# Guilucand/PanDelos

Measured on AMD Instinct MI355X. Metric: scored gene-pairs/sec (whole node), higher is better.
Workload: dtype u32 accumulate + f32 finalize

## Files before the change

### pandelos_amd/csrc/pdl_api.hip

```cpp
#include "pdl_common.h"

#include <algorithm>
#include <cstdlib>
#include <cstring>
#include <limits>

static thread_local std::string g_create_error = "";

#define PDL_GUARD_BEGIN try {
#define PDL_GUARD_END(ctx_)                                                       \
    } catch (const pdl_error &e) {                                                \
        if (ctx_) (ctx_)->err = e.msg; else g_create_error = e.msg;               \
        return e.code;                                                            \
    } catch (const std::bad_alloc &) {                                            \
        if (ctx_) (ctx_)->err = "host allocation failed";                         \
        return PDL_ERR_DEVICE;                                                    \
    }

template <class T> static T *xalloc(size_t n) {
    T *p = static_cast<T *>(malloc((n ? n : 1) * sizeof(T)));
    if (!p) throw std::bad_alloc();
    return p;
}

// ... 543 lines not shown
        if ((n_edges && (!src || !dst)) || (n_sequences && !genome_of)) PDL_FAIL(PDL_ERR_ARGUMENT, "pdl_families_of_edges: NULL pointer");
        if (n_edges >= 0x7fffffffull || n_sequences >= 0x7fffffffu) PDL_FAIL(PDL_ERR_UNSUPPORTED, "pdl_families_of_edges: 2^31 genes or edges and more");
        PDL_HIP(hipSetDevice(c->device));
        pdl_ctx::FamBufs &b = c->fb;
        uint32_t g_max = 0;
        for (uint32_t i = 0; i < n_sequences; i++) g_max = std::max(g_max, genome_of[i]);
        if (n_edges) {
            b.up_src.alloc(n_edges * 4); b.up_dst.alloc(n_edges * 4);
            PDL_HIP(hipMemcpyAsync(b.up_src.p, src, n_edges * 4, hipMemcpyHostToDevice, c->stream));
            PDL_HIP(hipMemcpyAsync(b.up_dst.p, dst, n_edges * 4, hipMemcpyHostToDevice, c->stream));
        }
        if (n_sequences) {
            b.up_gen.alloc((size_t) n_sequences * 4);
            PDL_HIP(hipMemcpyAsync(b.up_gen.p, genome_of, (size_t) n_sequences * 4, hipMemcpyHostToDevice, c->stream));
        }
        const int32_t *s2[2] = {b.up_src.as<int32_t>(), nullptr}, *d2[2] = {b.up_dst.as<int32_t>(), nullptr};
        const uint64_t n2[2] = {n_edges, 0};
        pdl_fam_result r;
        pdl_run_families(c, s2, d2, n2, false, true, true, b.up_gen.as<uint32_t>(), n_sequences, bit_length64(g_max), r);
        fill_families(r, out);
        return PDL_OK;
    } catch (const pdl_error &e) { c->err = e.msg; pdl_free_families(out); return e.code;
    } catch (const std::bad_alloc &) { c->err = "host allocation failed"; pdl_free_families(out); return PDL_ERR_DEVICE; }
}

int pdl_set_option(pdl_ctx *c, const char *name, int64_t value) {
    if (!c || !name) return PDL_ERR_ARGUMENT;
    std::lock_guard<std::mutex> lk(c->mu);
    const std::string n(name);
    if (n == "join_tier1") {
        if (!(value == -1 || value == 0 || (value >= 9 && value <= 11) || value == 20 || value == 21)) { c->err = "join_tier1: -1, 0, 9, 10, 11, 20 or 21"; return PDL_ERR_ARGUMENT; }
        c->opt_tier1 = (int) value;
    } else if (n == "join_tier0") c->opt_tier0 = value < 0 ? -1 : (value != 0);
    else if (n == "join_tiny_tier2") c->opt_tiny_tier2 = value != 0;
    else if (n == "join_grid_pct") c->opt_grid_pct = (int) value;
    else if (n == "stage_timers") c->opt_stage_timers = value != 0;
    else if (n == "host_mirror") c->opt_host_mirror = value != 0;
    else if (n == "staging_cap") c->opt_staging_cap = value > 0 ? (uint64_t) value : 0;
    else if (n == "aside_test_reload") c->opt_aside_test_reload = value != 0;
    else if (n == "onepass_scan") c->opt_onepass_scan = value != 0;
    else if (n == "low_memory") c->opt_low_memory = value != 0;
    else if (n == "query_batch_bytes") {
        if (value <= 0) { c->err = "query_batch_bytes: a positive byte count"; return PDL_ERR_ARGUMENT; }
        c->opt_query_batch_bytes = (uint64_t) value;
        return PDL_OK;
    }
    else { c->err = "unknown option " + n; return PDL_ERR_ARGUMENT; }
    c->scored = false;
    return PDL_OK;
}

int pdl_dist_preprocess_begin(pdl_ctx *c, const uint8_t *d_residues, const uint64_t *d_offsets, const uint32_t *d_genome_of,
                              uint32_t n, uint64_t n_res, int k, uint32_t world, uint32_t rank, pdl_dist_slice *out) {
    if (!c || !out) return PDL_ERR_ARGUMENT;
    std::lock_guard<std::mutex> lk(c->mu);
    PDL_GUARD_BEGIN
    if (!d_offsets || !d_genome_of || (!d_residues && n_res)) PDL_FAIL(PDL_ERR_ARGUMENT, "null input pointer");
    if (((uintptr_t) d_residues & 15) != 0) PDL_FAIL(PDL_ERR_ARGUMENT, "d_residues must be 16-byte aligned");
    if (world == 0 || rank >= world || world > 64) PDL_FAIL(PDL_ERR_ARGUMENT, "rank %u of %u (at most 64 ranks)", rank, world);
    PDL_HIP(hipSetDevice(c->device));
    c->preprocessed = false; c->scored = false; c->tasks_ready = false; c->mirror_valid = false;
    c->dist = false; c->dist_stage = 0;
    adopt_device_input(c, d_residues, d_offsets, d_genome_of, n, n_res);
    c->N = n; c->R = n_res;
    c->U = c->Ushared = c->NG = c->P = c->M = 0;
    if (k <= 0) PDL_FAIL(PDL_ERR_KVALUE, "K value must be greater than 0.");
// ... 281 lines not shown
```

### pandelos_amd/csrc/pdl_common.h

```cpp
#pragma once

#include <atomic>
#include <chrono>

#include <hip/hip_runtime.h>

#include <cstdint>
#include <cstdio>
#include <mutex>
#include <cstdlib>
#include <string>
#include <utility>
#include <vector>

#include "../../include/pandelos_amd.h"

#define PDL_WAVE 64

#ifdef __HIPCC__
__device__ __forceinline__ void pdl_sync() {
#ifndef PDL_PLAIN_SYNCTHREADS
    asm volatile("s_waitcnt lgkmcnt(0)" ::: "memory");
#endif
    __syncthreads();
// ... 227 lines not shown
    bool scored = false;
    uint32_t n_task_rows = 0;
    std::vector<int32_t> h_local_genome;
    std::vector<uint32_t> h_task_row_off;
    std::vector<uint64_t> h_cell_off;
    DevBuf task_blob;
    uint32_t *task_pin = nullptr; size_t task_pin_words = 0;
    hipStream_t copy_stream = nullptr; hipEvent_t ev_tasks = nullptr, ev_entry = nullptr;
    DevView task_rows;
    DevView task_lg;
    DevBuf row_desc;
    DevBuf MS;
    DevBuf CM;
    DevBuf row_base, row_cnt, fin_off;
    DevBuf st_score, st_perc, st_tr, st_col, st_first;
    uint64_t st_cap = 0;
    DevBuf c_score, c_perc, c_tr, c_row, c_col;
    uint64_t Z = 0;
    DevBuf join_ctr;
    DevBuf overflow_rows;
    DevBuf gene_info;
    DevBuf join_defer;
    DevBuf glb_table;
    bool glb_clean = false;
    DevBuf row_desc2;
    DevBuf mirror_cnt, mirror_ref;
    DevView taskpos_of;
    std::vector<uint32_t> h_fin;
    bool tasks_ready = false;
    DevBuf scratch2;
    DevBuf task_off;
    int cus = 0;
    uint32_t occ_tier1[5] = {0, 0, 0, 0, 0};
    uint32_t occ_tier0 = 0, occ_tier0b = 0;

    bool edges_valid = false;
    DevBuf bbh_kind, bbh_tab, e_src, e_dst, e_score;
    uint8_t *edge_mirror = nullptr;
    size_t edge_mirror_bytes = 0;
    uint64_t n_edges = 0, n_edges1 = 0;
    std::vector<uint32_t> h_bbh_at;
    std::vector<uint64_t> h_edge1, h_edge_off;

    int opt_tier1 = -1;
    int opt_tier0 = -1;
    bool opt_tiny_tier2 = false;
    bool opt_stage_timers = true;
    int opt_grid_pct = 0;
    bool opt_host_mirror = true;
    uint64_t opt_staging_cap = 0;
    bool opt_aside_test_reload = false;

    bool dist = false;
    uint32_t world = 1, rank = 0;
    int dist_stage = 0;
    uint2 *post_ext = nullptr;
    uint64_t U_slice = 0, M_slice = 0;
    std::vector<uint32_t> h_owner;
    std::vector<uint64_t> h_upper_cost;
    std::vector<uint64_t> h_run_weights;
    std::vector<uint64_t> h_run_costs;
    bool dist_sender = false;
    int dist_tail = -1;
    uint64_t run_base = 0, dist_total = 0;
    DevBuf seq_owner;
    DevBuf tuple_off;
    std::vector<uint64_t> h_tuple_counts;
    uint32_t *dist_out_keys = nullptr;
    unsigned long long *dist_out_ranges = nullptr;
    uint64_t dist_out_total = 0, dist_run_counters[3] = {0, 0, 0};
    DevBuf owner_of_genome;
    DevView local_genome;
    DevBuf outbox;
    DevBuf outbox_tab;
    std::vector<uint64_t> h_outbox_counts;
    uint64_t st_local = 0;
    uint64_t n_inbox = 0;
    uint32_t order_grid1 = 0;
// ... 226 lines not shown
```

### pandelos_amd/csrc/pdl_join.hip

```cpp
#include "pdl_common.h"
#include "pdl_scan.h"

#include <algorithm>
#include <cstdlib>
#include <cstring>

constexpr int HBM_THREADS = 512;
constexpr uint32_t EMPTY_KEY = 0xffffffffu;
constexpr uint64_t FIELD_MASK = (1ull << 21) - 1;
constexpr uint32_t CELL_CHUNK = 16384;

struct JoinArgs {
    const uint2 *post;
    const uint4 *ranges;
    const uint2 *ranges8;
    const uint32_t *seq_off;
    const uint32_t *kseq_len;
    const uint32_t *genome_of;
    const uint4 *gene_info;
    const uint32_t *task_rows;
    const uint32_t *task_lg;
    const uint32_t *work;
    const uint4 *desc;
    uint32_t n_work;
    const uint32_t *n_work_ptr;
    uint32_t N, G, k;
    uint32_t min_kseq;
    uint32_t canonical;
    float *MS;
    float *CM;
    uint32_t *row_base, *row_cnt;
    float *st_score, *st_perc, *st_tr;
    uint32_t *st_col, *st_first;
    uint32_t mirror;
    const uint32_t *taskpos_of;
    const uint32_t *local_genome;
    uint32_t *mirror_cnt;
    unsigned long long st_cap;
    uint32_t *work_cursor;
    uint32_t work_batch;
    unsigned long long *cell_cursor;
    uint32_t *overflow_count;
    uint32_t *error_count;
    uint32_t *overflow_rows;
    uint4 *overflow_desc;
#ifdef PDL_JOIN_PHASES
    unsigned long long *phase;
#endif
    void *defer;
    uint32_t defer_wide;
    uint32_t defer_cap;
    uint32_t *reload_count;
    uint32_t defer_serial;
    unsigned long long *hbm_acc;
    uint32_t *hbm_u32;
};

__device__ __forceinline__ uint32_t min_numerator(float threshold, float denom) {
    uint32_t n = (uint32_t) (threshold * denom);
    n = n > 2 ? n - 2 : 0;
    while ((float) (int) n / denom < threshold) n++;
    return n;
}

__device__ __forceinline__ float finalize_counts(int inter, int pc, int tc, uint32_t my_kcnt, uint32_t other_kcnt, float threshold,
                                                 float &perc, float &tr_perc) {
    const int union_size = (int) my_kcnt + (int) other_kcnt - inter;
    perc = (float) pc / (float) (int) my_kcnt;
    tr_perc = (float) tc / (float) (int) other_kcnt;
    const bool score_valid = perc >= threshold || tr_perc >= threshold;
    return (float) inter / (float) union_size * (score_valid ? 1.0f : 0.0f);
}
__device__ __forceinline__ float finalize_cell(unsigned long long acc, uint32_t my_kcnt, uint32_t other_kcnt, float threshold,
// ... 1098 lines not shown
        const uint32_t g = c->shard[i];
        c->h_local_genome[g] = (int32_t) i;
        c->h_task_row_off[i] = p;
        for (uint32_t j = c->h_genome_row_off[g]; j < c->h_genome_row_off[g + 1]; j++) { const uint32_t gene = c->h_genome_rows[j]; h_rows[p] = gene; h_lg[p] = i; h_pos[gene] = p; p++; }
    }
    for (uint32_t g = 0; g < G; g++) h_loc[g] = (uint32_t) c->h_local_genome[g];
    c->h_task_row_off[S] = n_rows;
    c->n_task_rows = n_rows;
    c->tasks_ready = true;
    if (!c->copy_stream) {
        PDL_HIP(hipStreamCreateWithFlags(&c->copy_stream, hipStreamNonBlocking));
        PDL_HIP(hipEventCreateWithFlags(&c->ev_tasks, hipEventDisableTiming));
    }
    memcpy(c->task_pin + words, c->h_task_row_off.data(), (size_t) (S + 1) * 4);
    c->task_blob.alloc(words * sizeof(uint32_t) + 16);
    if (n_rows) c->task_off.alloc((size_t) (S + 1) * 8 + 96);
    PDL_HIP(hipMemcpyAsync(c->task_blob.p, c->task_pin, words * sizeof(uint32_t), hipMemcpyHostToDevice, c->copy_stream));
    if (n_rows) PDL_HIP(hipMemcpyAsync(c->task_off.p, c->task_pin + words, (size_t) (S + 1) * 4, hipMemcpyHostToDevice, c->copy_stream));
    PDL_HIP(hipEventRecord(c->ev_tasks, c->copy_stream));
    PDL_HIP(hipStreamWaitEvent(st, c->ev_tasks, 0));
    uint32_t *d = c->task_blob.as<uint32_t>();
    c->task_rows.p = d; c->task_lg.p = d + n_rows; c->taskpos_of.p = d + 2 * (size_t) n_rows; c->local_genome.p = d + 2 * (size_t) n_rows + N;
    if (c->dist) {
        c->owner_of_genome.alloc((size_t) G * 4);
        PDL_HIP(hipMemcpyAsync(c->owner_of_genome.p, c->h_owner.data(), (size_t) G * 4, hipMemcpyHostToDevice, st));
    }
}

__global__ void k_iota_u32(uint32_t *dst, uint32_t n) { uint32_t i = blockIdx.x * blockDim.x + threadIdx.x; if (i < n) dst[i] = i; }

struct ScorePlan {
    bool wide, mirror;
    bool tier0;
    uint32_t grid0, grid0b;
    int tier1, occ_slot;
    bool tiny_tier2;
    uint32_t grid1, grid2, grid3;
    unsigned long long slack;
    bool wide_aside;
};

static ScorePlan score_plan(pdl_ctx *c) {
    const uint32_t N = c->N, G = c->G;
    const uint32_t n_rows = c->n_task_rows;
    const uint32_t S = (uint32_t) c->shard.size();
    ScorePlan pl{};
    pl.wide = c->max_kseq >= (1ull << 20);
    if (c->max_kseq >= (1ull << 31)) PDL_FAIL(PDL_ERR_UNSUPPORTED, "a gene with %llu k-mers exceeds the reference's int counters", (unsigned long long) c->max_kseq);
    pl.mirror = c->upper_only;
    if (pl.mirror && !c->dist && (c->shard_set && S != G))
        PDL_FAIL(PDL_ERR_STATE, "the dictionary was built for all genomes (upper-triangle ranges); a genome shard must be set before pdl_preprocess");
    const int cus = pdl_cus(c);
    pl.tier1 = c->opt_tier1 >= 0 ? c->opt_tier1 : (G <= 320 ? 10 : 11);
    pl.tiny_tier2 = c->opt_tiny_tier2;
    auto occupancy = [&](const void *fn, int threads) {
        int nb = 0;
        if (hipOccupancyMaxActiveBlocksPerMultiprocessor(&nb, fn, threads, 0) != hipSuccess || nb < 1) nb = 1;
        return (uint32_t) nb;
    };
    const int tier1 = pl.tier1;
    const void *fn1 = tier1 == 9 ? (const void *) k_join_lds<9, 128, true>
                    : tier1 == 10 ? (const void *) k_join_lds<10, 256, true>
                    : tier1 == 11 ? (const void *) k_join_lds<11, 256, true>
                    : tier1 == 20 ? (const void *) k_join_lds<10, 256, false> : (const void *) k_join_lds<11, 256, false>;
    const int t1_threads = tier1 == 9 ? 128 : 256;
    pl.occ_slot = tier1 >= 20 ? tier1 - 20 + 3 : (tier1 ? tier1 - 9 : 0);
    if (tier1 && c->occ_tier1[pl.occ_slot] == 0) c->occ_tier1[pl.occ_slot] = occupancy(fn1, t1_threads);
    pl.grid1 = tier1 ? std::min<uint32_t>(n_rows, (uint32_t) cus * c->occ_tier1[pl.occ_slot]) : 0;
    if (c->opt_grid_pct > 0 && pl.grid1) pl.grid1 = std::max<uint32_t>(1, (uint32_t) ((uint64_t) pl.grid1 * (uint32_t) c->opt_grid_pct / 100));
    {
        const unsigned long long walked = c->dist ? [&] { unsigned long long u = 0; for (uint32_t g : c->shard) u += c->h_upper_cost[g]; return u; }()
                                          : pl.mirror ? (c->P - c->Ushared) / 2 : c->P;
        const bool can = c->ranges8 != nullptr && !pl.wide && c->min_kseq > 2ull * c->rp.k && tier1 != 0;
        const bool want = c->opt_tier0 > 0 || (c->opt_tier0 < 0 && c->opt_tier1 < 0 && n_rows >= 12288 && walked / n_rows <= 3000 && c->Urepeat * 5000 <= c->U);
        pl.tier0 = can && want;
        if (pl.tier0) {
            if (c->occ_tier0 == 0) { c->occ_tier0 = occupancy((const void *) k_join_part<PT_T, PT_WG_PER_CU>, (int) PT_T); c->occ_tier0b = occupancy((const void *) k_join_part<PT_T2, PT_WGS2>, (int) PT_T2); }
            pl.grid0 = std::min<uint32_t>((n_rows + PT_BATCH - 1) / PT_BATCH, (uint32_t) cus * c->occ_tier0);
            pl.grid0b = std::min<uint32_t>(n_rows, (uint32_t) cus * c->occ_tier0b);
            if (c->opt_grid_pct > 0) pl.grid0 = std::max<uint32_t>(1, (uint32_t) ((uint64_t) pl.grid0 * (uint32_t) c->opt_grid_pct / 100));
        }
    }
    pl.grid2 = std::min<uint32_t>(n_rows, (uint32_t) cus * (pl.tiny_tier2 ? 4 : 1));
    {
        const unsigned long long per_wg = (unsigned long long) std::max<uint32_t>(N, 1) * ((pl.wide ? 2 : 1) * sizeof(uint64_t) + 3 * sizeof(uint32_t));
        const unsigned long long fit = ((c->opt_low_memory ? 1ull : 8ull) << 30) / per_wg;
        pl.grid3 = (uint32_t) std::min<unsigned long long>((unsigned long long) cus, std::max<unsigned long long>(64, fit));
    }
    const size_t hbm_bytes = (size_t) pl.grid3 * N * ((pl.wide ? 2 : 1) * sizeof(uint64_t) + 3 * sizeof(uint32_t));
    if (c->glb_table.bytes < hbm_bytes) { c->glb_table.alloc(hbm_bytes); c->glb_clean = false; }
    if (!c->glb_clean) {
        PDL_HIP(hipMemsetAsync(c->glb_table.p, 0, hbm_bytes, c->stream));
        c->glb_clean = true;
    }
    pl.slack = 2ull * (pl.grid0 + pl.grid0b + pl.grid1 + pl.grid2 + pl.grid3) * CELL_CHUNK;
    return pl;
}

static void score_alloc_rows(pdl_ctx *c, const ScorePlan &pl) {
    const uint32_t N = c->N, G = c->G, n_rows = c->n_task_rows;
    const uint32_t S = (uint32_t) c->shard.size();
    c->MS.alloc((size_t) n_rows * G * sizeof(float) + 16);
    c->CM.alloc((size_t) S * N * sizeof(float) + 16);
    c->row_base.alloc((size_t) n_rows * 4); c->row_cnt.alloc((size_t) n_rows * 4); c->fin_off.alloc(((size_t) n_rows + 2) * 4);
    c->join_ctr.alloc(PDL_JC_WORDS * sizeof(uint32_t));
    c->row_desc.alloc((size_t) n_rows * sizeof(uint4));
    c->row_desc2.alloc((size_t) n_rows * sizeof(uint4) * (pl.tier0 ? 3 : 1));
    c->overflow_rows.alloc((size_t) n_rows * 4 * 4);
    if (pl.mirror) c->mirror_cnt.alloc((size_t) n_rows * 4 * 3 + 16);
    c->gene_info.alloc((size_t) N * sizeof(uint4));
    hipLaunchKernelGGL(k_row_desc, dim3((std::max(n_rows, N) + 255) / 256), dim3(256), 0, c->stream, c->task_rows.as<uint32_t>(), c->seq_off.as<uint32_t>(),
                       n_rows, c->row_desc.as<uint4>(), c->kseq_len.as<uint32_t>(), c->d_gen, c->taskpos_of.as<uint32_t>(), c->local_genome.as<uint32_t>(),
                       N, c->gene_info.as<uint4>());
}

static void score_alloc_cells(pdl_ctx *c, const ScorePlan &pl, unsigned long long cap, unsigned long long extra) {
    const unsigned long long fcap = pl.mirror ? 2 * cap + extra : cap;
    if (fcap >= 0xffffffffull) PDL_FAIL(PDL_ERR_UNSUPPORTED, "more than 2^32 emitted cells on one device: shard the genomes over more devices");
    DevBuf *st[5] = {&c->st_score, &c->st_perc, &c->st_tr, &c->st_col, &c->st_first};
    for (int i = 0; i < 5; i++) st[i]->alloc(cap * 4);
    c->c_score.alloc(fcap * 4); c->c_perc.alloc(fcap * 4); c->c_tr.alloc(fcap * 4); c->c_row.alloc(fcap * 4); c->c_col.alloc(fcap * 4);
    if (pl.mirror) c->mirror_ref.alloc((cap + extra) * sizeof(MCell));
    c->st_cap = cap;
}

static JoinArgs join_args(pdl_ctx *c, const ScorePlan &pl) {
    JoinArgs a{};
    a.post = pdl_postings(c); a.ranges = c->ranges.as<uint4>(); a.ranges8 = c->ranges8; a.seq_off = c->seq_off.as<uint32_t>();
    a.kseq_len = c->kseq_len.as<uint32_t>(); a.genome_of = c->d_gen; a.gene_info = c->gene_info.as<uint4>();
    a.task_rows = c->task_rows.as<uint32_t>(); a.task_lg = c->task_lg.as<uint32_t>();
    a.N = c->N; a.G = c->G; a.k = c->rp.k;
    a.min_kseq = (uint32_t) std::max<uint64_t>(c->min_kseq, 1); a.canonical = (c->flags & PDL_FLAG_CANONICAL_ORDER) ? 1u : 0u;
    a.MS = c->MS.as<float>(); a.CM = c->CM.as<float>();
    a.row_base = c->row_base.as<uint32_t>(); a.row_cnt = c->row_cnt.as<uint32_t>();
    a.st_score = c->st_score.as<float>(); a.st_perc = c->st_perc.as<float>(); a.st_tr = c->st_tr.as<float>();
    a.st_col = c->st_col.as<uint32_t>(); a.st_first = c->st_first.as<uint32_t>(); a.st_cap = c->st_cap;
    a.mirror = pl.mirror ? 1u : 0u;
    if (pl.mirror) {
        a.taskpos_of = c->taskpos_of.as<uint32_t>(); a.local_genome = c->local_genome.as<uint32_t>();
        a.mirror_cnt = c->mirror_cnt.as<uint32_t>();
    }
    return a;
}

static void score_join(pdl_ctx *c, const ScorePlan &pl) {
    hipStream_t st = c->stream;
    const uint32_t N = c->N, G = c->G, n_rows = c->n_task_rows;
    const uint32_t S = (uint32_t) c->shard.size();
    const int tier1 = pl.tier1;
    {
        auto n16 = [](size_t bytes) { return (unsigned long long) ((bytes + 15) / 16); };
        ZeroRanges z{};
        z.p[0] = c->MS.as<uint4>(); z.n16[0] = n16((size_t) n_rows * G * sizeof(float));
        z.p[1] = c->CM.as<uint4>(); z.n16[1] = n16((size_t) S * N * sizeof(float));
        z.p[2] = c->join_ctr.as<uint4>(); z.n16[2] = n16(PDL_JC_WORDS * sizeof(uint32_t));
        z.p[3] = pl.mirror ? c->mirror_cnt.as<uint4>() : nullptr; z.n16[3] = pl.mirror ? n16((size_t) n_rows * 4 * 3) : 0;
        const unsigned long long most = std::max(z.n16[0], z.n16[1]);
        hipLaunchKernelGGL(k_zero_ranges, dim3((uint32_t) std::min<unsigned long long>((most + 255) / 256 + 1, (unsigned long long) c->cus * 16)), dim3(256), 0, st, z);
    }
    JoinArgs a = join_args(c, pl);
    uint32_t *ctr32 = c->join_ctr.as<uint32_t>();
    uint32_t *list_a = c->overflow_rows.as<uint32_t>(), *list_b = list_a + n_rows, *list_s = list_b + n_rows, *list_s2 = list_s + n_rows;
    a.error_count = ctr32 + PDL_JC_ERRORS; a.reload_count = ctr32 + PDL_JC_RELOADS;
    a.cell_cursor = reinterpret_cast<unsigned long long *>(ctr32 + PDL_JC_CELLS);

    ev_begin(c, EV_JOIN);
    if (pl.wide) {
        hipLaunchKernelGGL(k_iota_u32, dim3((n_rows + 255) / 256), dim3(256), 0, st, list_b, n_rows);
        PDL_HIP(hipMemcpyAsync(ctr32 + PDL_JC_ROWS_T3, &c->n_task_rows, 4, hipMemcpyHostToDevice, st));
    }
    a.work = nullptr; a.desc = c->row_desc.as<uint4>(); a.n_work = pl.wide ? 0 : n_rows; a.n_work_ptr = nullptr;
    if (pl.tier0) {
        a.work_cursor = ctr32 + PDL_JC_CURSOR_T0; a.overflow_count = ctr32 + PDL_JC_ROWS_T0B; a.overflow_rows = list_s; a.work_batch = PT_BATCH;
        a.overflow_desc = c->row_desc2.as<uint4>() + n_rows;
#ifdef PDL_JOIN_PHASES
        static unsigned long long *d_phase0 = nullptr;
        if (!d_phase0) PDL_HIP(hipMalloc((void **) &d_phase0, 12 * sizeof(unsigned long long)));
        PDL_HIP(hipMemsetAsync(d_phase0, 0, 12 * sizeof(unsigned long long), st));
        a.phase = d_phase0;
#endif
        hipLaunchKernelGGL((k_join_part<PT_T, PT_WG_PER_CU>), dim3(pl.grid0), dim3(PT_T), 0, st, a);
#ifdef PDL_JOIN_PHASES
        {
            unsigned long long h[12];
            PDL_HIP(hipMemcpyAsync(h, d_phase0, sizeof(h), hipMemcpyDeviceToHost, st));
            PDL_HIP(hipStreamSynchronize(st));
            const double per = 10.0 / 1000.0 / std::max<uint32_t>(pl.grid0, 1);
            fprintf(stderr, "tier 0 phases per workgroup (us): draw + pick %.1f  stage %.1f  prefixes %.1f  walk %.1f  sift + add %.1f  finalize %.1f  | rows/wg %.1f\n",
                    h[0] * per, h[1] * per, h[2] * per, h[3] * per, h[4] * per, h[5] * per, (double) n_rows / std::max<uint32_t>(pl.grid0, 1));
            fprintf(stderr, "tier 0 counts: cycles %llu (%.2f rows, %.0f lookups each)  cycles that overflowed %llu  survivors of wave 0 %llu (x4 = %.1f %% of the lookups)  probe steps of thread 0: %llu\n",
                    h[6], (double) h[11] / std::max<unsigned long long>(h[6], 1), (double) h[10] / std::max<unsigned long long>(h[6], 1), h[7], h[8], 400.0 * h[8] / std::max<unsigned long long>(h[10], 1), h[9]);
            a.phase = nullptr;
        }
#endif
        a.desc = c->row_desc2.as<uint4>() + n_rows; a.n_work = 0; a.n_work_ptr = ctr32 + PDL_JC_ROWS_T0B;
        a.work_cursor = ctr32 + PDL_JC_CURSOR_T0B; a.overflow_count = ctr32 + PDL_JC_ROWS_T1; a.overflow_rows = list_s2; a.work_batch = 1;
        a.overflow_desc = c->row_desc2.as<uint4>() + 2 * (size_t) n_rows;
        hipLaunchKernelGGL((k_join_part<PT_T2, PT_WGS2>), dim3(pl.grid0b), dim3(PT_T2), 0, st, a);
        a.desc = c->row_desc2.as<uint4>() + 2 * (size_t) n_rows; a.n_work = 0; a.n_work_ptr = ctr32 + PDL_JC_ROWS_T1;
        c->tm.join_launches += 2;
    }
    a.work_cursor = ctr32 + PDL_JC_CURSOR_T1; a.overflow_count = ctr32 + PDL_JC_ROWS_T2; a.overflow_rows = list_a; a.overflow_desc = tier1 ? c->row_desc2.as<uint4>() : nullptr;
    a.work_batch = pl.tier0 ? 1 : std::max<uint32_t>(1, std::min<uint32_t>(8, n_rows / (std::max<uint32_t>(pl.grid1, 1) * 8)));
    if (tier1 >= 9 && tier1 <= 11) {
        const unsigned long long avg = n_rows ? c->P / n_rows : 0;
        a.defer_cap = (uint32_t) std::min<unsigned long long>(std::min<unsigned long long>(std::max<unsigned long long>(4 * avg, 8192), 1u << 18), (unsigned long long) N + 64);
        a.defer_wide = (N >= (1u << 22) || pl.wide_aside) ? 1u : 0u;
        c->join_defer.alloc((size_t) pl.grid1 * a.defer_cap * (a.defer_wide ? sizeof(uint4) : sizeof(uint2)));
        a.defer = c->join_defer.p;
        static std::atomic<uint32_t> launch_serial{0};
        a.defer_serial = ++launch_serial;
    }
#ifdef PDL_JOIN_PHASES
    static unsigned long long *d_phase = nullptr;
    if (!d_phase) PDL_HIP(hipMalloc((void **) &d_phase, 10 * sizeof(unsigned long long)));
    PDL_HIP(hipMemsetAsync(d_phase, 0, 10 * sizeof(unsigned long long), st));
    a.phase = d_phase;
#endif
    if (tier1 == 9) hipLaunchKernelGGL((k_join_lds<9, 128, true>), dim3(pl.grid1), dim3(128), 0, st, a);
    else if (tier1 == 10) hipLaunchKernelGGL((k_join_lds<10, 256, true>), dim3(pl.grid1), dim3(256), 0, st, a);
    else if (tier1 == 11) hipLaunchKernelGGL((k_join_lds<11, 256, true>), dim3(pl.grid1), dim3(256), 0, st, a);
    else if (tier1 == 20) hipLaunchKernelGGL((k_join_lds<10, 256, false>), dim3(pl.grid1), dim3(256), 0, st, a);
    else if (tier1 == 21) hipLaunchKernelGGL((k_join_lds<11, 256, false>), dim3(pl.grid1), dim3(256), 0, st, a);
#ifdef PDL_JOIN_PHASES
    {
        unsigned long long h[10];
        PDL_HIP(hipMemcpyAsync(h, d_phase, sizeof(h), hipMemcpyDeviceToHost, st));
        PDL_HIP(hipStreamSynchronize(st));
        const double per = 10.0 / 1000.0 / std::max<uint32_t>(pl.grid1, 1);
        fprintf(stderr, "join phases per workgroup (us): dispense %.1f  stage %.1f  [walk: map %.1f  postings %.1f  bitmap %.1f  table %.1f  aside stores %.1f]  barrier %.1f  aside pass %.1f  finalize %.1f  | rows/wg %.1f\n",
                h[0] * per, h[1] * per, h[5] * per, h[6] * per, h[7] * per, h[8] * per, h[9] * per, h[2] * per, h[3] * per, h[4] * per,
// ... 267 lines not shown
```

### pandelos_amd/csrc/pdl_join_part.h

```cpp
#pragma once

constexpr uint32_t PT_T = 256;
constexpr uint32_t PT_T2 = 512, PT_WGS2 = 3;
constexpr uint32_t PT_RB = 960;
constexpr uint32_t PT_ROWS = 4;
#ifndef PT_WG_PER_CU
#define PT_WG_PER_CU 5
#endif
constexpr uint32_t PT_NCH = 4, PT_ITERS = PT_WG_PER_CU >= 5 ? 4 : 6;
constexpr uint32_t PT_KPT = PT_NCH * PT_ITERS;
constexpr uint32_t PT_HEAVY_CAP = 64;
constexpr uint32_t PT_BM_BITS = PT_WG_PER_CU >= 5 ? 10 : 11, PT_BM_WORDS = 1u << PT_BM_BITS;
constexpr uint32_t PT_BM_SHIFT = 22 - PT_BM_BITS;
constexpr uint32_t PT_HT_BITS = 10, PT_HT = 1u << PT_HT_BITS;
constexpr uint32_t PT_BATCH = 8;
constexpr uint32_t PT_HASH_MUL = 0x9E3779B1u & 0x3fffffu;
constexpr uint32_t pt_inverse(uint32_t m) { uint32_t x = m; for (int i = 0; i < 5; i++) x *= 2u - m * x; return x; }
constexpr uint32_t PT_HASH_INV = pt_inverse(PT_HASH_MUL);
static_assert((uint32_t) (PT_HASH_MUL * PT_HASH_INV) == 1u, "multiplicative inverse mod 2^32 (hence mod 2^22)");
static_assert(PT_RB <= 1022 && PT_RB % PDL_WAVE == 0 && (3 * PT_HT) / 4 + PT_T2 <= CELL_CHUNK, "10-bit range index");

__device__ __forceinline__ uint32_t pt_mul_u24(uint32_t a, uint32_t b) {
    uint32_t r;
    asm("v_mul_u32_u24 %0, %1, %2" : "=v"(r) : "v"(a), "v"(b));
    return r;
}

struct PartRow { uint32_t p, r, kcnt, genome, lg, pc_min, pad0, pad1; };

template <uint32_t TT, uint32_t WGS>
__global__ __launch_bounds__(TT, WGS) void k_join_part(JoinArgs a) {
    constexpr uint32_t PT_T = TT, PT_NW = PT_T / PDL_WAVE;
    constexpr uint32_t PT_RPT = (PT_RB + PT_T - 1) / PT_T;
    constexpr uint32_t PT_LMAX = PT_KPT * PT_T;
    constexpr uint32_t PT_WLIST = (PT_BM_WORDS + PT_RB + 66) / PT_NW;
    constexpr uint32_t PT_TOUCH_CAP = (3 * PT_HT) / 4 + PT_T;
    static_assert(PT_WLIST >= PT_NCH * PDL_WAVE, "a wave's list holds at least one round of survivors");
    __shared__ uint32_t s_big[2 * PT_BM_WORDS + PT_RB + 66];
    __shared__ uint32_t s_tkey[PT_HT];
    __shared__ uint32_t s_tn[PT_HT];
    __shared__ uint16_t s_touched[PT_TOUCH_CAP];
    __shared__ uint2 s_gm[PT_RB + 1];
    __shared__ uint2 s_heavy[PT_HEAVY_CAP];
    __shared__ uint4 s_bdesc[PT_BATCH], s_binfo[PT_BATCH];
    __shared__ PartRow s_row[PT_ROWS];
    __shared__ uint32_t s_wave[PT_NW];
    __shared__ uint2 s_lb[PT_ROWS + 1];
    __shared__ uint2 s_wstart[PT_NW];
    __shared__ uint32_t s_nheavy, s_ntouched, s_overflow, s_solo, s_tslot[PT_ROWS], s_nemit[PT_ROWS], s_w0, s_bn, s_bpos;
    __shared__ unsigned long long s_base, s_chunk_next, s_chunk_end;

    const uint32_t tid = threadIdx.x, lane = tid & (PDL_WAVE - 1), wave = tid / PDL_WAVE;
    const uint32_t n_work = a.n_work_ptr ? *a.n_work_ptr : a.n_work;
    if (n_work == 0) return;
    const uint32_t batch = min(max(a.work_batch, 1u), PT_BATCH);
    uint32_t *s_bm2 = s_big, *s_bm1 = s_big + PT_BM_WORDS, *s_cum = s_big + 2 * PT_BM_WORDS;
    for (uint32_t i = tid; i < PT_HT; i += PT_T) { s_tkey[i] = 0; s_tn[i] = 0; }
    if (tid == 0) { s_nheavy = 0; s_ntouched = 0; s_overflow = 0; s_solo = 0; s_bn = 0; s_bpos = 0; s_chunk_next = 0; s_chunk_end = 0; }
    if (tid < PT_ROWS) { s_tslot[tid] = 0; s_nemit[tid] = 0; }
    const float threshold = 1.0f / (2.0f * (float) a.k);
    const uint32_t tc_min = min_numerator(threshold, (float) (int) a.min_kseq);
    const bool track_first = a.canonical == 0;
    const uint32_t two_k = 2 * a.k;
#ifdef PDL_JOIN_PHASES
    unsigned long long pph[6] = {0, 0, 0, 0, 0, 0}, pt_prev = wall_clock64();
    unsigned long long pt_cycles = 0, pt_over = 0, pt_surv = 0, pt_probe = 0, pt_look = 0, pt_rows = 0;
#define PT_MARK(i) do { if (tid == 0) { const unsigned long long t_now = wall_clock64(); pph[i] += t_now - pt_prev; pt_prev = t_now; } } while (0)
#else
#define PT_MARK(i) do { } while (0)
#endif

    for (;;) {
        pdl_sync();
        PT_MARK(5);
        if (s_bpos >= s_bn) {
            if (tid == 0) s_w0 = atomicAdd(a.work_cursor, batch);
            pdl_sync();
            const uint32_t w0 = s_w0;
            if (w0 >= n_work) break;
            if (tid < batch && w0 + tid < n_work) {
                const uint4 d = a.desc[w0 + tid];
                s_bdesc[tid] = d;
                s_binfo[tid] = a.gene_info[d.y];
            }
            if (tid == 0) { s_bn = min(batch, n_work - w0); s_bpos = 0; }
            pdl_sync();
        }
        const uint32_t bn = (uint32_t) __builtin_amdgcn_readfirstlane((int) s_bn);
        uint32_t j = (uint32_t) __builtin_amdgcn_readfirstlane((int) s_bpos);
// ... 7 lines not shown
        }
        if (j >= bn) { pdl_sync(); if (tid == 0) s_bpos = j; continue; }
        PT_MARK(0);
        const bool solo = uni(s_solo) != 0;
        uint32_t ns = 0, nb = 0, rbv[PT_ROWS + 1], e0v[PT_ROWS], jv[PT_ROWS];
        {
            bool stop = false;
#pragma unroll
            for (uint32_t s = 0; s < PT_ROWS; s++) {
                rbv[s] = nb; e0v[s] = 0; jv[s] = j;
                if (!stop && j < bn && (s == 0 || !solo)) {
                    const uint4 d = s_bdesc[j];
                    const uint32_t dw = uni(d.w), kc = uni(s_binfo[j].x);
                    if (dw == 0 || dw > PT_RB || kc <= two_k || nb + dw > PT_RB) stop = true;
                    else { e0v[s] = uni(d.z); nb += dw; ns = s + 1; j++; }
                }
            }
            rbv[PT_ROWS] = nb;
#pragma unroll
            for (uint32_t s = 0; s < PT_ROWS; s++) if (s >= ns) rbv[s] = nb;
        }
        uint32_t len[PT_RPT], sum = 0;
        {
            uint2 rg[PT_RPT];
#pragma unroll
            for (uint32_t q = 0; q < PT_RPT; q++) {
                const uint32_t i = min(tid * PT_RPT + q, nb - 1);
                const uint32_t s = (uint32_t) (i >= rbv[1]) + (uint32_t) (i >= rbv[2]) + (uint32_t) (i >= rbv[3]);
                const uint32_t e0 = s == 0 ? e0v[0] : s == 1 ? e0v[1] : s == 2 ? e0v[2] : e0v[3];
                const uint32_t rb = s == 0 ? rbv[0] : s == 1 ? rbv[1] : s == 2 ? rbv[2] : rbv[3];
                rg[q] = a.ranges8[e0 + (i - rb)];
            }
#pragma unroll
            for (uint32_t i = 0; i < 2 * PT_BM_WORDS / 4 / PT_T; i++) reinterpret_cast<uint4 *>(s_big)[i * PT_T + tid] = make_uint4(0, 0, 0, 0);
#pragma unroll
            for (uint32_t q = 0; q < PT_RPT; q++) {
                const uint32_t i = tid * PT_RPT + q;
                len[q] = 0;
                if (i < nb) { s_gm[i] = rg[q]; len[q] = rg[q].y & 0x3fffffu; }
                sum += len[q];
            }
        }
        const uint32_t inc = wave_inclusive_scan_u32(sum);
        if (lane == PDL_WAVE - 1) s_wave[wave] = inc;
        {
            uint32_t ex_w = inc - sum;
#pragma unroll
            for (uint32_t q = 0; q < PT_RPT; q++) {
                const uint32_t i = tid * PT_RPT + q;
#pragma unroll
                for (uint32_t s = 1; s < PT_ROWS; s++) if (s < ns && i == rbv[s]) s_lb[s] = make_uint2(wave, ex_w);
                ex_w += len[q];
            }
        }
        pdl_sync();
        PT_MARK(1);
        uint32_t woff[PT_NW + 1];
        woff[0] = 0;
#pragma unroll
        for (uint32_t w = 0; w < PT_NW; w++) woff[w + 1] = woff[w] + uni(s_wave[w]);
        uint32_t lbv[PT_ROWS + 1];
        lbv[0] = 0;
#pragma unroll
        for (uint32_t s = 1; s < PT_ROWS; s++) {
            lbv[s] = woff[PT_NW];
            if (s < ns) { const uint2 v = s_lb[s]; const uint32_t vx = uni(v.x); uint32_t wo = 0;
#pragma unroll
// ... 46 lines not shown
            if (placed) {
                atomicMin(&s_tkey[tbase + ts], k1);
                atomicAdd(&s_tn[tbase + ts], 1u);
            } else s_overflow = 1;
        };
        const uint32_t chunks = (total + PDL_WAVE - 1) / PDL_WAVE;
        const uint32_t cpw = (chunks + PT_NW - 1) / PT_NW;
        const uint32_t seg = cpw * PDL_WAVE;
        {
            uint32_t ex = inc - sum;
#pragma unroll
            for (uint32_t w = 0; w < PT_NW; w++) ex += wave == w ? woff[w] : 0u;
#pragma unroll
            for (uint32_t q = 0; q < PT_RPT; q++) {
                const uint32_t i = tid * PT_RPT + q;
                if (i < PT_RB) s_cum[i] = i < nbk ? ex : (i == nbk ? total : 0xffffffffu);
                if (len[q] && i < nbk) {
                    uint32_t w_lo = 0;
#pragma unroll
                    for (uint32_t w = 0; w < PT_NW; w++) w_lo += (uint32_t) (w * seg < ex);
                    for (uint32_t w = w_lo; w < PT_NW && w * seg < ex + len[q]; w++) s_wstart[w] = make_uint2(i, ex);
                }
                ex += len[q];
            }
            for (uint32_t i = PT_RB + tid; i < PT_RB + 66; i += PT_T) s_cum[i] = i == nbk ? total : 0xffffffffu;
            if (tid < PT_ROWS && tid < ns_keep) {
                const uint32_t jj = tid == 0 ? jv[0] : tid == 1 ? jv[1] : tid == 2 ? jv[2] : jv[3];
                const uint4 d = s_bdesc[jj], inf = s_binfo[jj];
                s_row[tid] = PartRow{d.x, d.y, inf.x, inf.y, inf.w, min_numerator(threshold, (float) (int) inf.x), 0u, 0u};
            }
        }
        pdl_sync();
        PT_MARK(2);
        uint32_t key[PT_KPT];
#pragma unroll
        for (uint32_t i = 0; i < PT_KPT; i++) key[i] = 0xffffffffu;
        const uint32_t ch0 = wave * cpw;
        {
            uint32_t ch = ch0;
            const uint32_t ch_end = min(chunks, ch + cpw);
            const uint2 ws = s_wstart[wave];
            uint32_t rs = (uint32_t) __builtin_amdgcn_readfirstlane((int) ws.x);
#pragma unroll
            for (uint32_t it = 0; it < PT_ITERS; it++) {
                if (ch < ch_end) {
                    uint2 po[PT_NCH];
                    uint32_t adr[PT_NCH];
                    bool live[PT_NCH];
                    uint32_t ownhv = 0;
                    const uint32_t nu = min(PT_NCH, ch_end - ch);
                    const uint32_t f_lo = ch * PDL_WAVE, f_hi = f_lo + nu * PDL_WAVE;
                    const uint32_t vw = s_cum[rs + 1 + lane];
                    if ((uint32_t) __builtin_amdgcn_readlane((int) vw, PDL_WAVE - 1) >= f_hi) {
#pragma unroll
                        for (uint32_t u = 0; u < PT_NCH; u++) {
                            live[u] = false; adr[u] = 0; key[it * PT_NCH + u] = 0;
                            if (u < nu) {
                                const uint32_t lo = f_lo + u * PDL_WAVE, f = lo + lane;
                                const uint32_t cu = (uint32_t) __popcll(__ballot(vw <= lo));
                                const bool inside = vw > lo && vw < lo + PDL_WAVE;
                                const int recv = __builtin_amdgcn_ds_permute((int) ((inside ? vw - lo : 0u) << 2), inside ? 1 : 0);
                                const unsigned long long m = __ballot(recv != 0);
                                const uint32_t r = rs + cu + __builtin_amdgcn_mbcnt_hi((uint32_t) (m >> 32), __builtin_amdgcn_mbcnt_lo((uint32_t) m, 0u)) + (uint32_t) (recv != 0);
                                live[u] = f < total;
                                const uint32_t rl = live[u] ? r : 0u;
                                const uint2 gmu = s_gm[rl];
// ... 2 lines not shown
                                adr[u] = gmu.x + (f - cum_r);

                                ownhv |= (uint32_t) ((gmu.y >> 22) >= 2u) << u;
                            }
                        }
                        const uint32_t ce = (uint32_t) __popcll(__ballot(vw <= f_hi));
                        rs += ce;
                    } else {
#pragma unroll
                        for (uint32_t u = 0; u < PT_NCH; u++) {
                            live[u] = false; adr[u] = 0; key[it * PT_NCH + u] = 0;
                            if (u < nu) {
                                const uint32_t f0 = (ch + u) * PDL_WAVE, f = f0 + lane;
                                const uint32_t v = s_cum[rs + 1 + lane];
                                const bool inside = v < f0 + PDL_WAVE;
                                const int recv = __builtin_amdgcn_ds_permute((int) ((inside ? v - f0 : 0u) << 2), inside ? 1 : 0);
                                const unsigned long long m = __ballot(recv != 0);
                                const uint32_t w = (uint32_t) __popcll(__ballot(inside));
                                const uint32_t r = rs + __builtin_amdgcn_mbcnt_hi((uint32_t) (m >> 32), __builtin_amdgcn_mbcnt_lo((uint32_t) m, 0u)) + (uint32_t) (recv != 0);
                                live[u] = f < total;
                                const uint32_t rl = live[u] ? r : 0u;
                                const uint2 gmu = s_gm[rl];
                                const uint32_t cum_r = s_cum[rl];
                                key[it * PT_NCH + u] = rl;
                                adr[u] = gmu.x + (f - cum_r);
                                ownhv |= (uint32_t) ((gmu.y >> 22) >= 2u) << u;
                                const uint32_t nextb = w < PDL_WAVE ? (uint32_t) __builtin_amdgcn_readlane((int) v, w) : s_cum[rs + 1 + PDL_WAVE];
                                rs += w + (uint32_t) (nextb == f0 + PDL_WAVE);
                            }
                        }
                    }
#pragma unroll
                    for (uint32_t u = 0; u < PT_NCH; u++) po[u] = a.post[live[u] ? adr[u] : 0u];
                    uint32_t seen[PT_NCH], bit[PT_NCH], wd[PT_NCH];
#pragma unroll
                    for (uint32_t u = 0; u < PT_NCH; u++) {
                        const uint32_t h = pt_mul_u24(po[u].x, PT_HASH_MUL) & 0x3fffffu;
                        key[it * PT_NCH + u] |= h << 10;
                        wd[u] = h >> PT_BM_SHIFT; bit[u] = 1u << ((h >> (PT_BM_SHIFT - 5)) & 31u);
                        seen[u] = live[u] ? atomicOr(&s_bm1[wd[u]], bit[u]) : 0u;
                        if (live[u] && (po[u].y >= 2u || ((ownhv >> u) & 1u))) {
                            seen[u] = bit[u];
                            const uint32_t i = atomicAdd(&s_nheavy, 1u);
                            if (i < PT_HEAVY_CAP) s_heavy[i] = make_uint2(key[it * PT_NCH + u], po[u].y);
                        }
                    }
#pragma unroll
                    for (uint32_t u = 0; u < PT_NCH; u++) if (seen[u] & bit[u]) atomicOr(&s_bm2[wd[u]], bit[u]);
                }
                ch += PT_NCH;
            }
        }
        pdl_sync();
        PT_MARK(3);
        uint32_t *wlist = s_bm1 + wave * PT_WLIST;
        uint32_t nsv = 0;
        const uint32_t n_heavy = uni(s_nheavy);
        if (n_heavy > PT_HEAVY_CAP) s_overflow = 1;
        auto drain = [&]() {
            asm volatile("s_waitcnt lgkmcnt(0)" ::: "memory");
            for (uint32_t i0 = 0; i0 < nsv; i0 += 2 * PDL_WAVE) {
                const uint32_t ia = i0 + lane, ib = ia + PDL_WAVE;
                const uint32_t ka = wlist[ia < nsv ? ia : 0u], kb = wlist[ib < nsv ? ib : 0u];
                if (ia < nsv) add_one(ka);
                if (ib < nsv) add_one(kb);
            }
            nsv = 0;
        };
        {
            const uint32_t nkeys = ch0 < chunks ? min(chunks - ch0, cpw) : 0u;
#pragma unroll
            for (uint32_t g = 0; g < PT_ITERS; g++) {
                if (g * PT_NCH >= nkeys) break;
                if (nsv + PT_NCH * PDL_WAVE > PT_WLIST) drain();
                uint32_t twice[PT_NCH];
#pragma unroll
                for (uint32_t u = 0; u < PT_NCH; u++) twice[u] = s_bm2[(key[g * PT_NCH + u] >> (10 + PT_BM_SHIFT)) & (PT_BM_WORDS - 1)];
#pragma unroll
                for (uint32_t u = 0; u < PT_NCH; u++) {
                    const uint32_t i = g * PT_NCH + u;
                    if (i >= nkeys) break;
                    const bool keep = (ch0 + i) * PDL_WAVE + lane < total && ((twice[u] >> ((key[i] >> (10 + PT_BM_SHIFT - 5)) & 31u)) & 1u);
                    const unsigned long long mk = __ballot(keep);
                    if (keep) wlist[nsv + (uint32_t) __popcll(mk & ((1ull << lane) - 1ull))] = key[i];
                    nsv += (uint32_t) __popcll(mk);
#ifdef PDL_JOIN_PHASES
                    if (tid == 0) pt_surv += (uint32_t) __popcll(mk);
#endif
                }
            }
            drain();
        }
        pdl_sync();
        PT_MARK(4);
#ifdef PDL_JOIN_PHASES
        if (tid == 0) { pt_cycles++; pt_look += total; pt_rows += ns_keep; if (uni(s_overflow)) pt_over++; }
#endif
        if (uni(s_overflow)) {
            pdl_sync();
            for (uint32_t i = tid; i < PT_HT; i += PT_T) { s_tkey[i] = 0; s_tn[i] = 0; }
            const bool hand_on = ns_keep == 1;
            if (tid == 0 && hand_on) { const uint4 d = s_bdesc[jv[0]]; const uint32_t oi = atomicAdd(a.overflow_count, 1u); a.overflow_rows[oi] = d.x; a.overflow_desc[oi] = d; }
            if (tid < PT_ROWS) s_tslot[tid] = 0;
            if (tid == 0) {
                s_nheavy = 0; s_ntouched = 0; s_overflow = 0;
                s_solo = hand_on ? (solo ? uni(s_solo) - 1u : 0u) : ns_keep;
                s_bpos = hand_on ? next_pos : jv[0];
            }
            continue;
        }
        const uint32_t ntouched = min(uni(s_ntouched), PT_TOUCH_CAP);
        if (tid == 0) {
            unsigned long long nx = s_chunk_next;
            if (nx + ntouched > s_chunk_end) {
                nx = atomicAdd(a.cell_cursor, (unsigned long long) CELL_CHUNK);
                s_chunk_end = nx + CELL_CHUNK;
            }
            s_base = nx;
        }
        pdl_sync();
        const unsigned long long base = s_base;
        const bool fits = base + ntouched <= a.st_cap;
        const uint32_t c0 = uni(s_tslot[0]), c1 = uni(s_tslot[1]), c2 = uni(s_tslot[2]);
        const uint32_t sb1 = c0, sb2 = c0 + c1, sb3 = c0 + c1 + c2;
// ... 71 lines not shown
```

Baseline: 1329 billion.

## Replace seen-twice bitmaps with 16-bit counting sieve using score threshold

```diff
diff --git a/pandelos_amd/csrc/pdl_api.hip b/pandelos_amd/csrc/pdl_api.hip
--- a/pandelos_amd/csrc/pdl_api.hip
+++ b/pandelos_amd/csrc/pdl_api.hip
@@ -599,6 +599,10 @@
         if (!(value == -1 || value == 0 || (value >= 9 && value <= 11) || value == 20 || value == 21)) { c->err = "join_tier1: -1, 0, 9, 10, 11, 20 or 21"; return PDL_ERR_ARGUMENT; }
         c->opt_tier1 = (int) value;
     } else if (n == "join_tier0") c->opt_tier0 = value < 0 ? -1 : (value != 0);
+    else if (n == "sift_threshold") {
+        if (value != 0 && value != 1) { c->err = "sift_threshold: 0 or 1"; return PDL_ERR_ARGUMENT; }
+        c->opt_sift_threshold = (int) value;
+    }
     else if (n == "join_tiny_tier2") c->opt_tiny_tier2 = value != 0;
     else if (n == "join_grid_pct") c->opt_grid_pct = (int) value;
     else if (n == "stage_timers") c->opt_stage_timers = value != 0;
diff --git a/pandelos_amd/csrc/pdl_common.h b/pandelos_amd/csrc/pdl_common.h
--- a/pandelos_amd/csrc/pdl_common.h
+++ b/pandelos_amd/csrc/pdl_common.h
@@ -283,7 +283,7 @@
     DevBuf task_off;
     int cus = 0;
     uint32_t occ_tier1[5] = {0, 0, 0, 0, 0};
-    uint32_t occ_tier0 = 0, occ_tier0b = 0;
+    uint32_t occ_tier0[2] = {0, 0}, occ_tier0b[2] = {0, 0};
 
     bool edges_valid = false;
     DevBuf bbh_kind, bbh_tab, e_src, e_dst, e_score;
@@ -295,6 +295,7 @@
 
     int opt_tier1 = -1;
     int opt_tier0 = -1;
+    int opt_sift_threshold = 1;
     bool opt_tiny_tier2 = false;
     bool opt_stage_timers = true;
     int opt_grid_pct = 0;
diff --git a/pandelos_amd/csrc/pdl_join.hip b/pandelos_amd/csrc/pdl_join.hip
--- a/pandelos_amd/csrc/pdl_join.hip
+++ b/pandelos_amd/csrc/pdl_join.hip
@@ -39,6 +39,7 @@
     unsigned long long st_cap;
     uint32_t *work_cursor;
     uint32_t work_batch;
+    uint32_t sift_threshold;
     unsigned long long *cell_cursor;
     uint32_t *overflow_count;
     uint32_t *error_count;
@@ -1203,6 +1204,7 @@
 struct ScorePlan {
     bool wide, mirror;
     bool tier0;
+    bool tier0_cnt;
     uint32_t grid0, grid0b;
     int tier1, occ_slot;
     bool tiny_tier2;
@@ -1246,9 +1248,20 @@
         const bool want = c->opt_tier0 > 0 || (c->opt_tier0 < 0 && c->opt_tier1 < 0 && n_rows >= 12288 && walked / n_rows <= 3000 && c->Urepeat * 5000 <= c->U);
         pl.tier0 = can && want;
         if (pl.tier0) {
-            if (c->occ_tier0 == 0) { c->occ_tier0 = occupancy((const void *) k_join_part<PT_T, PT_WG_PER_CU>, (int) PT_T); c->occ_tier0b = occupancy((const void *) k_join_part<PT_T2, PT_WGS2>, (int) PT_T2); }
-            pl.grid0 = std::min<uint32_t>((n_rows + PT_BATCH - 1) / PT_BATCH, (uint32_t) cus * c->occ_tier0);
-            pl.grid0b = std::min<uint32_t>(n_rows, (uint32_t) cus * c->occ_tier0b);
+            {
+                const float thr = 1.0f / (2.0f * (float) c->rp.k), denom = (float) (int) (uint32_t) std::max<uint64_t>(c->min_kseq, 1);
+                uint32_t t = (uint32_t) (thr * denom);
+                t = t > 2 ? t - 2 : 0;
+                while ((float) (int) t / denom < thr) t++;
+                pl.tier0_cnt = c->opt_sift_threshold == 0 || t >= PT_SIFT_T_MIN;
+            }
+            const int f = pl.tier0_cnt ? 1 : 0;
+            if (c->occ_tier0[f] == 0) {
+                c->occ_tier0[f] = f ? occupancy((const void *) k_join_part<PT_T, PT_WG_PER_CU, true>, (int) PT_T) : occupancy((const void *) k_join_part<PT_T, PT_WG_PER_CU, false>, (int) PT_T);
+                c->occ_tier0b[f] = f ? occupancy((const void *) k_join_part<PT_T2, PT_WGS2, true>, (int) PT_T2) : occupancy((const void *) k_join_part<PT_T2, PT_WGS2, false>, (int) PT_T2);
+            }
+            pl.grid0 = std::min<uint32_t>((n_rows + PT_BATCH - 1) / PT_BATCH, (uint32_t) cus * c->occ_tier0[f]);
+            pl.grid0b = std::min<uint32_t>(n_rows, (uint32_t) cus * c->occ_tier0b[f]);
             if (c->opt_grid_pct > 0) pl.grid0 = std::max<uint32_t>(1, (uint32_t) ((uint64_t) pl.grid0 * (uint32_t) c->opt_grid_pct / 100));
         }
     }
@@ -1307,6 +1320,7 @@
     a.st_score = c->st_score.as<float>(); a.st_perc = c->st_perc.as<float>(); a.st_tr = c->st_tr.as<float>();
     a.st_col = c->st_col.as<uint32_t>(); a.st_first = c->st_first.as<uint32_t>(); a.st_cap = c->st_cap;
     a.mirror = pl.mirror ? 1u : 0u;
+    a.sift_threshold = c->opt_sift_threshold ? 1u : 0u;
     if (pl.mirror) {
         a.taskpos_of = c->taskpos_of.as<uint32_t>(); a.local_genome = c->local_genome.as<uint32_t>();
         a.mirror_cnt = c->mirror_cnt.as<uint32_t>();
@@ -1350,7 +1364,8 @@
         PDL_HIP(hipMemsetAsync(d_phase0, 0, 12 * sizeof(unsigned long long), st));
         a.phase = d_phase0;
 #endif
-        hipLaunchKernelGGL((k_join_part<PT_T, PT_WG_PER_CU>), dim3(pl.grid0), dim3(PT_T), 0, st, a);
+        if (pl.tier0_cnt) hipLaunchKernelGGL((k_join_part<PT_T, PT_WG_PER_CU, true>), dim3(pl.grid0), dim3(PT_T), 0, st, a);
+        else hipLaunchKernelGGL((k_join_part<PT_T, PT_WG_PER_CU, false>), dim3(pl.grid0), dim3(PT_T), 0, st, a);
 #ifdef PDL_JOIN_PHASES
         {
             unsigned long long h[12];
@@ -1367,7 +1382,8 @@
         a.desc = c->row_desc2.as<uint4>() + n_rows; a.n_work = 0; a.n_work_ptr = ctr32 + PDL_JC_ROWS_T0B;
         a.work_cursor = ctr32 + PDL_JC_CURSOR_T0B; a.overflow_count = ctr32 + PDL_JC_ROWS_T1; a.overflow_rows = list_s2; a.work_batch = 1;
         a.overflow_desc = c->row_desc2.as<uint4>() + 2 * (size_t) n_rows;
-        hipLaunchKernelGGL((k_join_part<PT_T2, PT_WGS2>), dim3(pl.grid0b), dim3(PT_T2), 0, st, a);
+        if (pl.tier0_cnt) hipLaunchKernelGGL((k_join_part<PT_T2, PT_WGS2, true>), dim3(pl.grid0b), dim3(PT_T2), 0, st, a);
+        else hipLaunchKernelGGL((k_join_part<PT_T2, PT_WGS2, false>), dim3(pl.grid0b), dim3(PT_T2), 0, st, a);
         a.desc = c->row_desc2.as<uint4>() + 2 * (size_t) n_rows; a.n_work = 0; a.n_work_ptr = ctr32 + PDL_JC_ROWS_T1;
         c->tm.join_launches += 2;
     }
diff --git a/pandelos_amd/csrc/pdl_join_part.h b/pandelos_amd/csrc/pdl_join_part.h
--- a/pandelos_amd/csrc/pdl_join_part.h
+++ b/pandelos_amd/csrc/pdl_join_part.h
@@ -11,7 +11,13 @@
 constexpr uint32_t PT_KPT = PT_NCH * PT_ITERS;
 constexpr uint32_t PT_HEAVY_CAP = 64;
 constexpr uint32_t PT_BM_BITS = PT_WG_PER_CU >= 5 ? 10 : 11, PT_BM_WORDS = 1u << PT_BM_BITS;
+constexpr uint32_t PT_CNT_WORDS = 2 * PT_BM_WORDS;
+constexpr uint32_t PT_CNT_SHIFT = 22 - (PT_BM_BITS + 2);
+constexpr uint32_t PT_T_MAX = 255;
 constexpr uint32_t PT_BM_SHIFT = 22 - PT_BM_BITS;
+#ifndef PT_SIFT_T_MIN
+#define PT_SIFT_T_MIN 4
+#endif
 constexpr uint32_t PT_HT_BITS = 10, PT_HT = 1u << PT_HT_BITS;
 constexpr uint32_t PT_BATCH = 8;
 constexpr uint32_t PT_HASH_MUL = 0x9E3779B1u & 0x3fffffu;
@@ -19,6 +25,7 @@
 constexpr uint32_t PT_HASH_INV = pt_inverse(PT_HASH_MUL);
 static_assert((uint32_t) (PT_HASH_MUL * PT_HASH_INV) == 1u, "multiplicative inverse mod 2^32 (hence mod 2^22)");
 static_assert(PT_RB <= 1022 && PT_RB % PDL_WAVE == 0 && (3 * PT_HT) / 4 + PT_T2 <= CELL_CHUNK, "10-bit range index");
+static_assert(PT_KPT * PT_T2 + PT_HEAVY_CAP * PT_T_MAX < (1u << 16), "a 16-bit counter cannot overflow");
 
 __device__ __forceinline__ uint32_t pt_mul_u24(uint32_t a, uint32_t b) {
     uint32_t r;
@@ -28,15 +35,16 @@
 
 struct PartRow { uint32_t p, r, kcnt, genome, lg, pc_min, pad0, pad1; };
 
-template <uint32_t TT, uint32_t WGS>
+template <uint32_t TT, uint32_t WGS, bool CNT>
 __global__ __launch_bounds__(TT, WGS) void k_join_part(JoinArgs a) {
     constexpr uint32_t PT_T = TT, PT_NW = PT_T / PDL_WAVE;
     constexpr uint32_t PT_RPT = (PT_RB + PT_T - 1) / PT_T;
     constexpr uint32_t PT_LMAX = PT_KPT * PT_T;
-    constexpr uint32_t PT_WLIST = (PT_BM_WORDS + PT_RB + 66) / PT_NW;
+    constexpr uint32_t PT_LIST = !CNT || PT_RB + 66 > PT_NW * PT_NCH * PDL_WAVE ? PT_RB + 66 : PT_NW * PT_NCH * PDL_WAVE;
+    constexpr uint32_t PT_WLIST = (CNT ? PT_LIST : PT_BM_WORDS + PT_LIST) / PT_NW;
     constexpr uint32_t PT_TOUCH_CAP = (3 * PT_HT) / 4 + PT_T;
-    static_assert(PT_WLIST >= PT_NCH * PDL_WAVE, "a wave's list holds at least one round of survivors");
-    __shared__ uint32_t s_big[2 * PT_BM_WORDS + PT_RB + 66];
+    static_assert(PT_WLIST >= PT_NCH * PDL_WAVE && PT_NCH % 2 == 0, "a wave's list holds four rounds of survivors: room for two is made before every two");
+    __shared__ uint32_t s_big[PT_CNT_WORDS + PT_LIST];
     __shared__ uint32_t s_tkey[PT_HT];
     __shared__ uint32_t s_tn[PT_HT];
     __shared__ uint16_t s_touched[PT_TOUCH_CAP];
@@ -54,7 +62,8 @@
     const uint32_t n_work = a.n_work_ptr ? *a.n_work_ptr : a.n_work;
     if (n_work == 0) return;
     const uint32_t batch = min(max(a.work_batch, 1u), PT_BATCH);
-    uint32_t *s_bm2 = s_big, *s_bm1 = s_big + PT_BM_WORDS, *s_cum = s_big + 2 * PT_BM_WORDS;
+    uint32_t *s_cnt = s_big, *s_cum = s_big + PT_CNT_WORDS;
+    uint32_t *s_bm2 = s_big, *s_bm1 = s_big + PT_BM_WORDS;
     for (uint32_t i = tid; i < PT_HT; i += PT_T) { s_tkey[i] = 0; s_tn[i] = 0; }
     if (tid == 0) { s_nheavy = 0; s_ntouched = 0; s_overflow = 0; s_solo = 0; s_bn = 0; s_bpos = 0; s_chunk_next = 0; s_chunk_end = 0; }
     if (tid < PT_ROWS) { s_tslot[tid] = 0; s_nemit[tid] = 0; }
@@ -128,7 +137,7 @@
                 rg[q] = a.ranges8[e0 + (i - rb)];
             }
 #pragma unroll
-            for (uint32_t i = 0; i < 2 * PT_BM_WORDS / 4 / PT_T; i++) reinterpret_cast<uint4 *>(s_big)[i * PT_T + tid] = make_uint4(0, 0, 0, 0);
+            for (uint32_t i = 0; i < PT_CNT_WORDS / 4 / PT_T; i++) reinterpret_cast<uint4 *>(s_big)[i * PT_T + tid] = make_uint4(0, 0, 0, 0);
 #pragma unroll
             for (uint32_t q = 0; q < PT_RPT; q++) {
                 const uint32_t i = tid * PT_RPT + q;
@@ -241,6 +250,13 @@
         }
         pdl_sync();
         PT_MARK(2);
+        uint32_t sift_t = 2u;
+        if (CNT && a.sift_threshold) {
+            sift_t = tc_min;
+#pragma unroll
+            for (uint32_t s = 0; s < PT_ROWS; s++) if (s < ns_keep) sift_t = min(sift_t, uni(s_row[s].pc_min));
+            sift_t = min(max(sift_t, 2u), PT_T_MAX);
+        }
         uint32_t key[PT_KPT];
 #pragma unroll
         for (uint32_t i = 0; i < PT_KPT; i++) key[i] = 0xffffffffu;
@@ -309,6 +325,21 @@
                     }
 #pragma unroll
                     for (uint32_t u = 0; u < PT_NCH; u++) po[u] = a.post[live[u] ? adr[u] : 0u];
+                    if constexpr (CNT) {
+#pragma unroll
+                        for (uint32_t u = 0; u < PT_NCH; u++) {
+                            const uint32_t h = pt_mul_u24(po[u].x, PT_HASH_MUL) & 0x3fffffu;
+                            key[it * PT_NCH + u] |= h << 10;
+                            const uint32_t ci = h >> PT_CNT_SHIFT;
+                            uint32_t add = 1u;
+                            if (live[u] && (po[u].y >= 2u || ((ownhv >> u) & 1u))) {
+                                const uint32_t i = atomicAdd(&s_nheavy, 1u);
+                                add = i < PT_HEAVY_CAP ? sift_t : 0u;
+                                if (i < PT_HEAVY_CAP) s_heavy[i] = make_uint2(key[it * PT_NCH + u], po[u].y);
+                            }
+                            if (live[u]) atomicAdd(&s_cnt[ci >> 1], add << ((ci & 1u) << 4));
+                        }
+                    } else {
                     uint32_t seen[PT_NCH], bit[PT_NCH], wd[PT_NCH];
 #pragma unroll
                     for (uint32_t u = 0; u < PT_NCH; u++) {
@@ -324,40 +355,45 @@
                     }
 #pragma unroll
                     for (uint32_t u = 0; u < PT_NCH; u++) if (seen[u] & bit[u]) atomicOr(&s_bm2[wd[u]], bit[u]);
+                    }
                 }
                 ch += PT_NCH;
             }
         }
         pdl_sync();
         PT_MARK(3);
-        uint32_t *wlist = s_bm1 + wave * PT_WLIST;
+        uint32_t *wlist = (CNT ? s_cum : s_bm1) + wave * PT_WLIST;
         uint32_t nsv = 0;
         const uint32_t n_heavy = uni(s_nheavy);
         if (n_heavy > PT_HEAVY_CAP) s_overflow = 1;
-        auto drain = [&]() {
+        auto drain = [&](bool all) {
             asm volatile("s_waitcnt lgkmcnt(0)" ::: "memory");
-            for (uint32_t i0 = 0; i0 < nsv; i0 += 2 * PDL_WAVE) {
+            const uint32_t i_lo = all ? 0u : nsv % (2 * PDL_WAVE);
+            for (uint32_t i0 = i_lo; i0 < nsv; i0 += 2 * PDL_WAVE) {
                 const uint32_t ia = i0 + lane, ib = ia + PDL_WAVE;
                 const uint32_t ka = wlist[ia < nsv ? ia : 0u], kb = wlist[ib < nsv ? ib : 0u];
                 if (ia < nsv) add_one(ka);
                 if (ib < nsv) add_one(kb);
             }
-            nsv = 0;
+            nsv = i_lo;
         };
         {
             const uint32_t nkeys = ch0 < chunks ? min(chunks - ch0, cpw) : 0u;
 #pragma unroll
             for (uint32_t g = 0; g < PT_ITERS; g++) {
                 if (g * PT_NCH >= nkeys) break;
-                if (nsv + PT_NCH * PDL_WAVE > PT_WLIST) drain();
-                uint32_t twice[PT_NCH];
-#pragma unroll
-                for (uint32_t u = 0; u < PT_NCH; u++) twice[u] = s_bm2[(key[g * PT_NCH + u] >> (10 + PT_BM_SHIFT)) & (PT_BM_WORDS - 1)];
+                if (!CNT && nsv + PT_NCH * PDL_WAVE > PT_WLIST) drain(true);
+                uint32_t cw[PT_NCH];
+#pragma unroll
+                for (uint32_t u = 0; u < PT_NCH; u++)
+                    cw[u] = CNT ? s_cnt[(key[g * PT_NCH + u] >> (10 + PT_CNT_SHIFT + 1)) & (PT_CNT_WORDS - 1)] : s_bm2[(key[g * PT_NCH + u] >> (10 + PT_BM_SHIFT)) & (PT_BM_WORDS - 1)];
 #pragma unroll
                 for (uint32_t u = 0; u < PT_NCH; u++) {
                     const uint32_t i = g * PT_NCH + u;
                     if (i >= nkeys) break;
-                    const bool keep = (ch0 + i) * PDL_WAVE + lane < total && ((twice[u] >> ((key[i] >> (10 + PT_BM_SHIFT - 5)) & 31u)) & 1u);
+                    if (CNT && u % 2 == 0 && nsv + 2 * PDL_WAVE > PT_WLIST) drain(false);
+                    const bool keep = (ch0 + i) * PDL_WAVE + lane < total &&
+                                      (CNT ? ((cw[u] >> (((key[i] >> (10 + PT_CNT_SHIFT)) & 1u) << 4)) & 0xffffu) >= sift_t : ((cw[u] >> ((key[i] >> (10 + PT_BM_SHIFT - 5)) & 31u)) & 1u) != 0u);
                     const unsigned long long mk = __ballot(keep);
                     if (keep) wlist[nsv + (uint32_t) __popcll(mk & ((1ull << lane) - 1ull))] = key[i];
                     nsv += (uint32_t) __popcll(mk);
@@ -366,7 +402,7 @@
 #endif
                 }
             }
-            drain();
+            drain(true);
         }
         pdl_sync();
         PT_MARK(4);
```

Result: faster. 1437 billion, median of 6 (+8.1%).
